# SewoongLab/PLeaS-Merging

Measured on NVIDIA B200. Metric: rn50_pair_merge_calib_samples_per_s, higher is better.
Workload: dtype f32

## Files before the change

include/pleas_b200.h:

```cpp
#ifndef PLEAS_B200_H
#define PLEAS_B200_H

#include <stdint.h>

#ifdef __cplusplus
extern "C" {
#endif

#define PLB_OK 0
#define PLB_EINVAL (-1)
#define PLB_ESIZE (-2)
#define PLB_EALIGN (-3)

#define PLB_MODE_INNER 0
#define PLB_MODE_NEG_CDIST 1
#define PLB_MODE_CORR 2

int plb_version(void);
const char *plb_last_error_string(void);


int64_t plb_plane_bytes(int64_t rows, int64_t K, int32_t *row_groups, int32_t *k_blocks);

int plb_pack_split(const float *x, int64_t outer, int64_t src_rows, int64_t inner,
// ... 53 lines not shown
  const double *qa, *qb;
  const double *sa, *sb;
  int64_t ld_m, ld_n, K;
  int32_t splits;
  int32_t n_affine;
  const double *affine;
} PlbFinalizeTap;
typedef struct PlbFinalizeGroup {
  float *cost;
  int64_t ldc;
  int32_t n, tap_begin, tap_end, block_begin;
} PlbFinalizeGroup;
int plb_cross_finalize_grouped(const PlbFinalizeTap *taps_dev, const PlbFinalizeGroup *groups_dev,
                               int32_t n_groups, int32_t total_blocks, int32_t mode, int32_t accumulate,
                               void *stream);

int plb_cross_finalize_corr(const float *partial, int32_t splits, int64_t ld_m, int64_t ld_n,
                            int64_t M, int64_t N, const double *qa, const double *qb,
                            const double *sa, const double *sb, int64_t K, float *cost, int64_t ldc,
                            int32_t accumulate, void *stream);

int plb_lap_solve_batched(const float *const *cost, const int32_t *n, const int32_t *ld,
                          int64_t *const *col4row, double *objective, int32_t *status,
                          int32_t n_problems, int32_t max_n, int32_t maximize, void *stream);

int plb_lap_solve_batched_warm(const float *const *cost, const int32_t *n, const int32_t *ld,
                               int64_t *const *col4row, double *objective, int32_t *status,
                               int32_t n_problems, int32_t max_n, int32_t maximize,
                               const double *const *v_in, double v_scale, double *const *v_out, void *stream);


int plb_get_blocks(const float *cost, int64_t ldc, const int64_t *perm, int32_t n, float ratio,
                   int32_t identity, int64_t *q_merged, int64_t *p_merged, int64_t *q_sep,
                   int64_t *p_sep, int32_t *counts, void *stream);

int plb_block_merge(const float *w1, const float *w2, int64_t O, int64_t I, int64_t R,
                    const int64_t *bo1, const int64_t *bo2, const int64_t *bo1c, const int64_t *bo2c,
                    int64_t no, int64_t mo,
                    const int64_t *bi1, const int64_t *bi2, const int64_t *bi1c, const int64_t *bi2c,
                    int64_t ni, int64_t mi, int32_t in_axis_only, float *out, void *stream);

int plb_gather_axis(const float *in, float *out, int64_t outer, int64_t n, int64_t inner,
                    const int64_t *P, void *stream);

int plb_compose_perm(const int64_t *a, const int64_t *b, int64_t *out, int64_t n, void *stream);

int plb_wm_progress(const float *A, int64_t ld, const int64_t *P, int32_t n, int32_t *flag,
                    double *gain, void *stream);

int plb_conv_debug_set_trace(unsigned long long *dev_buf);
int64_t plb_conv_packed_floats(int64_t Cout, int64_t Cin, int32_t KH, int32_t KW);
int plb_conv_pack_weights(const float *w, int64_t Cout, int64_t Cin, int32_t KH, int32_t KW, float *packed,
                          void *stream);

int plb_conv2d_forward(const float *const *x, const float *const *packed_w, const float *const *bias,
                       float *const *out, int32_t nprob, int64_t NB, int64_t Cin, int64_t IH, int64_t IW,
                       int64_t Cout, int32_t KH, int32_t KW, int32_t stride, int32_t pad_h, int32_t pad_w,
                       void *stream);

int plb_conv2d_affine_forward(const float *const *x, const float *const *packed_w, const float *const *bias,
                              float *const *out, const float *const *scale_shift, float *const *out2,
                              int32_t relu, int32_t nprob, int64_t NB, int64_t Cin, int64_t IH, int64_t IW,
                              int64_t Cout, int32_t KH, int32_t KW, int32_t stride, int32_t pad_h, int32_t pad_w,
                              void *stream);

int plb_chol_solve(double *G, int64_t n, double *B, int64_t nrhs, double ridge, int32_t *info,
                   void *stream);

#ifdef __cplusplus
}
#endif
#endif
```

pleas_merging_b200/_native.py:

```python
import ctypes
import os

_HERE = os.path.dirname(os.path.abspath(__file__))
LIB_PATH = os.path.join(_HERE, "lib", "libpleas_b200.so")

c_i32, c_i64, c_f32, c_f64, c_ptr = ctypes.c_int32, ctypes.c_int64, ctypes.c_float, ctypes.c_double, ctypes.c_void_p


class GemmProblem(ctypes.Structure):
    _fields_ = [
        ("a_hi", c_ptr), ("a_lo", c_ptr), ("b_hi", c_ptr), ("b_lo", c_ptr), ("partial", c_ptr),
        ("a_row_groups", c_i32), ("b_row_groups", c_i32), ("k_blocks", c_i32),
        ("m_tiles", c_i32), ("n_tiles", c_i32), ("splits", c_i32), ("cta_begin", c_i32), ("symmetric", c_i32),
    ]


class FinalizeTap(ctypes.Structure):
    _fields_ = [("partial", c_ptr), ("qa", c_ptr), ("qb", c_ptr), ("sa", c_ptr), ("sb", c_ptr),
                ("ld_m", c_i64), ("ld_n", c_i64), ("K", c_i64), ("splits", c_i32), ("n_affine", c_i32),
                ("affine", c_ptr)]


class FinalizeGroup(ctypes.Structure):
    _fields_ = [("cost", c_ptr), ("ldc", c_i64), ("n", c_i32), ("tap_begin", c_i32), ("tap_end", c_i32),
                ("block_begin", c_i32)]


_SIGNATURES = {
    "plb_version": (ctypes.c_int, []),
    "plb_last_error_string": (ctypes.c_char_p, []),
    "plb_plane_bytes": (c_i64, [c_i64, c_i64, ctypes.POINTER(c_i32), ctypes.POINTER(c_i32)]),
    "plb_pack_split": (ctypes.c_int, [c_ptr, c_i64, c_i64, c_i64, c_ptr, c_i64, c_ptr, c_ptr, c_i32, c_i32,
                                      c_ptr, c_ptr, c_ptr]),
    "plb_pack_split_pair": (ctypes.c_int, [c_ptr, c_ptr, c_i64, c_i64, c_i64, c_ptr, c_ptr, c_ptr, c_ptr, c_i32, c_i32,
                                           c_ptr, c_ptr, c_ptr]),
    "plb_gram_direct": (ctypes.c_int, [c_ptr, c_ptr, c_i64, c_i64, c_i64, c_ptr, c_i32, c_i32, c_ptr, c_ptr, c_ptr]),
    "plb_gram_tma": (ctypes.c_int, [c_ptr, c_ptr, c_i64, c_i64, c_i64, c_ptr, c_i32, c_i32, c_ptr, c_ptr, c_ptr, c_ptr,
                                    c_ptr]),
    "plb_pack_split_pair_sums": (ctypes.c_int, [c_ptr, c_ptr, c_i64, c_i64, c_i64, c_ptr, c_ptr, c_ptr, c_ptr, c_i32,
                                                c_i32, c_ptr, c_ptr, c_ptr, c_ptr, c_ptr]),
    "plb_cross_finalize_grouped": (ctypes.c_int, [c_ptr, c_ptr, c_i32, c_i32, c_i32, c_i32, c_ptr]),
    "plb_cross_finalize_corr": (ctypes.c_int, [c_ptr, c_i32, c_i64, c_i64, c_i64, c_i64, c_ptr, c_ptr, c_ptr, c_ptr,
                                               c_i64, c_ptr, c_i64, c_i32, c_ptr]),
    "plb_gram_tma_geometry": (ctypes.c_int, [c_i64, ctypes.POINTER(c_i32), ctypes.POINTER(c_i32),
                                             ctypes.POINTER(c_i32), ctypes.POINTER(c_i32), ctypes.POINTER(c_i32)]),
    "plb_debug_set_trace": (ctypes.c_int, [c_ptr]),
    "plb_pack_im2col": (ctypes.c_int, [c_ptr, c_ptr, c_i64, c_i64, c_i64, c_i64, c_ptr, c_ptr, c_ptr, c_ptr, c_i64,
                                       c_i32, c_i32, c_i32, c_i32, c_i32, c_i32, c_i32, c_i32, c_i64, c_i64, c_i32,
                                       c_ptr, c_ptr, c_i32, c_i32, c_ptr]),
    "plb_gemm_grouped": (ctypes.c_int, [c_ptr, c_i32, c_i32, c_i32, c_i32, c_ptr]),
    "plb_cross_finalize": (ctypes.c_int, [c_ptr, c_i32, c_i64, c_i64, c_i64, c_i64, c_ptr, c_ptr, c_i32, c_ptr,
                                          c_ptr, c_i64, c_i32, c_i32, c_ptr]),
    "plb_lap_solve_batched": (ctypes.c_int, [c_ptr, c_ptr, c_ptr, c_ptr, c_ptr, c_ptr, c_i32, c_i32, c_i32, c_ptr]),
    "plb_lap_solve_batched_warm": (ctypes.c_int, [c_ptr, c_ptr, c_ptr, c_ptr, c_ptr, c_ptr, c_i32, c_i32, c_i32, c_ptr,
                                                  c_f64, c_ptr, c_ptr]),
    "plb_get_blocks": (ctypes.c_int, [c_ptr, c_i64, c_ptr, c_i32, c_f32, c_i32, c_ptr, c_ptr, c_ptr, c_ptr, c_ptr,
                                      c_ptr]),
    "plb_block_merge": (ctypes.c_int, [c_ptr, c_ptr, c_i64, c_i64, c_i64, c_ptr, c_ptr, c_ptr, c_ptr, c_i64, c_i64,
                                       c_ptr, c_ptr, c_ptr, c_ptr, c_i64, c_i64, c_i32, c_ptr, c_ptr]),
    "plb_gather_axis": (ctypes.c_int, [c_ptr, c_ptr, c_i64, c_i64, c_i64, c_ptr, c_ptr]),
    "plb_compose_perm": (ctypes.c_int, [c_ptr, c_ptr, c_ptr, c_i64, c_ptr]),
    "plb_wm_progress": (ctypes.c_int, [c_ptr, c_i64, c_ptr, c_i32, c_ptr, c_ptr, c_ptr]),
    "plb_chol_solve": (ctypes.c_int, [c_ptr, c_i64, c_ptr, c_i64, c_f64, c_ptr, c_ptr]),
    "plb_conv_debug_set_trace": (ctypes.c_int, [c_ptr]),
    "plb_conv_packed_floats": (c_i64, [c_i64, c_i64, c_i32, c_i32]),
    "plb_conv_pack_weights": (ctypes.c_int, [c_ptr, c_i64, c_i64, c_i32, c_i32, c_ptr, c_ptr]),
    "plb_conv2d_forward": (ctypes.c_int, [c_ptr, c_ptr, c_ptr, c_ptr, c_i32, c_i64, c_i64, c_i64, c_i64, c_i64,
                                          c_i32, c_i32, c_i32, c_i32, c_i32, c_ptr]),
    "plb_conv2d_affine_forward": (ctypes.c_int, [c_ptr, c_ptr, c_ptr, c_ptr, c_ptr, c_ptr, c_i32, c_i32, c_i64, c_i64,
                                                 c_i64, c_i64, c_i64, c_i32, c_i32, c_i32, c_i32, c_i32, c_ptr]),
}

EXPORTED_SYMBOLS = tuple(_SIGNATURES)
_lib = None


def lib():
    global _lib
    if _lib is None:
        if not os.path.exists(LIB_PATH):
            raise RuntimeError(
                f"pleas_merging_b200: CUDA library not found at {LIB_PATH}; build it with "
                "`python -m pleas_merging_b200.build` (or __graft_entry__.build()). There is no CPU fallback.")
        handle = ctypes.CDLL(LIB_PATH)
        for name, (res, args) in _SIGNATURES.items():
            fn = getattr(handle, name)
            fn.restype, fn.argtypes = res, args
        _lib = handle
    return _lib


import collections

LAUNCH_COUNTS = collections.Counter()


def check(rc, what):
    LAUNCH_COUNTS[what] += 1
    if rc != 0:
        msg = lib().plb_last_error_string().decode(errors="replace")
        raise RuntimeError(f"pleas_merging_b200: {what} failed with status {rc}: {msg}")


def call(name, device, *args):
    import torch

    fn = getattr(lib(), name)
    if device.index is None or device.index == torch.cuda.current_device():
        rc = fn(*args, torch.cuda.current_stream().cuda_stream)
    else:
        with torch.cuda.device(device):
            rc = fn(*args, torch.cuda.current_stream(device).cuda_stream)
    check(rc, name)


def stream_ptr(device=None):
    import torch

    return torch.cuda.current_stream(device).cuda_stream
# ... 17 lines not shown
```

pleas_merging_b200/csrc/conv.cu:

```cuda
#include "tma.cuh"

namespace plb {

constexpr int kConvStages = 4;
constexpr int kConvThreads = 576;
constexpr int kConvMaxFlatK = 512;

struct ConvParams {
  const float *x[2];
  const float *bias[2];
  float *out[2];
  const float2 *post[2];
  float *out2[2];
  int post_relu;
  int nprob;
  int NB, Cin, IH, IW, Cout, OH, OW, KH, KW, stride, pad_h, pad_w;
  int P, OHW, IHW;
  int m_tiles, n_tiles, total_items;
  int taps;
  int nbox;
  int flat;
  int flat_groups;
  int flat_lg;
  int chain_boxes;
  unsigned long long *trace;
  int debug;
};

__device__ __forceinline__ void tmem_st16(uint32_t taddr, const uint32_t (&v)[16]) {
  asm volatile(
      "tcgen05.st.sync.aligned.32x32b.x16.b32 [%0], "
      "{%1, %2, %3, %4, %5, %6, %7, %8, %9, %10, %11, %12, %13, %14, %15, %16};" ::"r"(taddr),
      "r"(v[0]), "r"(v[1]), "r"(v[2]), "r"(v[3]), "r"(v[4]), "r"(v[5]), "r"(v[6]), "r"(v[7]), "r"(v[8]), "r"(v[9]),
      "r"(v[10]), "r"(v[11]), "r"(v[12]), "r"(v[13]), "r"(v[14]), "r"(v[15])
      : "memory");
}
__device__ __forceinline__ void tmem_st_wait() { asm volatile("tcgen05.wait::st.sync.aligned;" ::: "memory"); }
__device__ __forceinline__ void tmem_ld16(uint32_t taddr, uint32_t (&v)[16]) {
  asm volatile(
      "tcgen05.ld.sync.aligned.32x32b.x16.b32 "
      "{%0, %1, %2, %3, %4, %5, %6, %7, %8, %9, %10, %11, %12, %13, %14, %15}, [%16];"
      : "=r"(v[0]), "=r"(v[1]), "=r"(v[2]), "=r"(v[3]), "=r"(v[4]), "=r"(v[5]), "=r"(v[6]), "=r"(v[7]),
        "=r"(v[8]), "=r"(v[9]), "=r"(v[10]), "=r"(v[11]), "=r"(v[12]), "=r"(v[13]), "=r"(v[14]), "=r"(v[15])
      : "r"(taddr));
}
__device__ __forceinline__ void umma_tf32_ts(uint32_t tmem_d, uint32_t tmem_a, uint64_t bdesc, uint32_t idesc,
                                             uint32_t accumulate) {
  asm volatile(
      "{\n\t.reg .pred p;\n\t"
      "setp.ne.b32 p, %4, 0;\n\t"
      "tcgen05.mma.cta_group::1.kind::tf32 [%0], [%1], %2, %3, p;\n\t}" ::"r"(tmem_d),
      "r"(tmem_a), "l"(bdesc), "r"(idesc), "r"(accumulate)
      : "memory");
}
__device__ __forceinline__ void tma_load_4d(void *smem_dst, const CUtensorMap *map, int c0, int c1, int c2, int c3,
                                            uint64_t *bar) {
  asm volatile(
      "cp.async.bulk.tensor.4d.shared::cluster.global.tile.mbarrier::complete_tx::bytes [%0], [%1, {%2, %3, %4, %5}], "
      "[%6];" ::"r"(smem_u32(smem_dst)),
      "l"(map), "r"(c0), "r"(c1), "r"(c2), "r"(c3), "r"(smem_u32(bar))
      : "memory");
}

template <int TN>
struct ConvCfg {
  static constexpr int kBBytes = kConvStages * 2 * TN * 128;
  static constexpr int kARing = TN == 128 ? 5 : 8;
  static constexpr int kSmemBytes = kBBytes + kARing * 16384 + 1024;
};

__device__ __forceinline__ void cp_async4(uint32_t smem_dst, const float *src, uint32_t ignore) {
  asm volatile(
      "{\n\t.reg .pred p;\n\t"
      "setp.ne.b32 p, %2, 0;\n\t"
      "cp.async.ca.shared.global [%0], [%1], 4, p;\n\t}" ::"r"(smem_dst),
      "l"(src), "r"(ignore)
      : "memory");
}
__device__ __forceinline__ void cp_async_commit() { asm volatile("cp.async.commit_group;" ::: "memory"); }
template <int N>
__device__ __forceinline__ void cp_async_wait() {
  asm volatile("cp.async.wait_group %0;" ::"n"(N) : "memory");
}

__device__ __forceinline__ uint32_t opaque_smem_u32(const void *p) {
  uint32_t a;
  asm volatile("{\n\t.reg .u64 t;\n\tcvta.to.shared.u64 t, %1;\n\tcvt.u32.u64 %0, t;\n\t}" : "=r"(a) : "l"(p));
  return a;
}
__device__ __forceinline__ void a32_expect_tx(uint32_t bar, uint32_t bytes) {
  asm volatile("mbarrier.arrive.expect_tx.shared::cta.b64 _, [%0], %1;" ::"r"(bar), "r"(bytes) : "memory");
}
__device__ __forceinline__ void a32_arrive(uint32_t bar) {
  asm volatile("mbarrier.arrive.shared::cta.b64 _, [%0];" ::"r"(bar) : "memory");
}
__device__ __forceinline__ bool a32_try_wait(uint32_t bar, uint32_t parity) {
  uint32_t ok;
  asm volatile(
      "{\n\t.reg .pred P;\n\t"
      "mbarrier.try_wait.parity.shared::cta.b64 P, [%1], %2;\n\t"
      "selp.b32 %0, 1, 0, P;\n\t}"
      : "=r"(ok)
      : "r"(bar), "r"(parity)
      : "memory");
  return ok != 0;
}
__device__ __forceinline__ bool a32_test_wait(uint32_t bar, uint32_t parity) {
  uint32_t ok;
  asm volatile(
      "{\n\t.reg .pred P;\n\t"
      "mbarrier.test_wait.parity.shared::cta.b64 P, [%1], %2;\n\t"
      "selp.b32 %0, 1, 0, P;\n\t}"
      : "=r"(ok)
      : "r"(bar), "r"(parity)
      : "memory");
  return ok != 0;
}
__device__ __forceinline__ void a32_wait_wd(uint32_t bar, uint32_t parity) {
  if (a32_try_wait(bar, parity)) return;
  const long long t0 = clock64();
  while (!a32_try_wait(bar, parity))
    if (clock64() - t0 > kWatchdogClocks) __trap();
// ... 19 lines not shown
    const int2 e = rows[r];
    const bool rowok = pvalid && e.y >= 0 && (unsigned)(ih0 + e.y) < (unsigned)IH;
    const float *base = rowok ? origin + e.x : safe;
#pragma unroll
    for (int t = 0; t < TAPS; ++t) {
      const bool ok = rowok && t < KW && (unsigned)(iw0 + t) < (unsigned)IW;
      cp_async4(dst + (r * TAPS + t) * 512, base + (ok ? t : 0), ok ? 0u : 1u);
    }
  }
}

template <int COLS, bool BIAS, bool POST>
__device__ __forceinline__ void store_tile(const float (&acc)[COLS], float *o, float *o2, int ohw, const float *bias,
                                           const float2 *ss, bool relu, int) {
#pragma unroll
  for (int c = 0; c < COLS; ++c) {
    const float v = acc[c];
    o[(int64_t)c * ohw] = v;
    if (POST) {
      const float2 a = __ldg(ss + c);
      const float w = fmaf(v, a.x, a.y);
      o2[(int64_t)c * ohw] = relu ? fmaxf(w, 0.f) : w;
    }
  }
}
template <int COLS>
__device__ __noinline__ void store_tile_ragged(const float (&acc)[COLS], float *o, float *o2, int ohw, const float *bias,
                                               const float2 *ss, bool relu, int nc) {
#pragma unroll 4
  for (int c = 0; c < COLS; ++c) {
    if (c >= nc) break;
    const float v = acc[c] + (bias ? __ldg(bias + c) : 0.f);
    o[(int64_t)c * ohw] = v;
    if (o2 != nullptr) {
      const float2 a = __ldg(ss + c);
      const float w = fmaf(v, a.x, a.y);
      o2[(int64_t)c * ohw] = relu ? fmaxf(w, 0.f) : w;
    }
  }
}

struct ConvItem {
  int prob, mt, nt;
};
__device__ __forceinline__ ConvItem conv_item(const ConvParams &p, int item) {
  ConvItem it;
  it.nt = item % p.n_tiles;
  const int rest = item / p.n_tiles;
  it.prob = rest % p.nprob;
  it.mt = rest / p.nprob;
  return it;
}

template <int TN, int CH, bool DBG>
__global__ void __launch_bounds__(kConvThreads, 1) conv3xtf32_kernel(const __grid_constant__ CUtensorMap tmw0,
                                                                      const __grid_constant__ CUtensorMap tmw1,
                                                                      ConvParams p) {
  constexpr int kPlaneBytes = TN * 128;
  constexpr int kStageBytes = 2 * kPlaneBytes;
  constexpr uint32_t kACol0 = 2 * TN;
  constexpr int kARing = ConvCfg<TN>::kARing;
  extern __shared__ uint8_t smem_raw[];
  __shared__ uint64_t bars[2 * kConvStages + 4];
  __shared__ uint32_t tmem_base_s;
  __shared__ int2 ktab[kConvMaxFlatK];

  uint8_t *smem = (uint8_t *)(((uintptr_t)smem_raw + 1023) & ~(uintptr_t)1023);
  const int warp = threadIdx.x >> 5, lane = threadIdx.x & 31;
  const int cta = (int)blockIdx.x, nctas = (int)gridDim.x;
  const uint32_t bars_a = opaque_smem_u32(bars), smem_a = opaque_smem_u32(smem);
  const uint32_t bar_full = bars_a, bar_empty = bars_a + 8 * kConvStages, bar_acc_full = bars_a + 16 * kConvStages,
                 bar_acc_empty = bar_acc_full + 16;

  if (warp == 0 && lane == 0) {
    for (int s = 0; s < kConvStages; ++s) {
      mbar_init(&bars[s], 1 + 8);
      mbar_init(&bars[kConvStages + s], 1);
    }
    for (int b = 0; b < 2; ++b) {
      mbar_init(&bars[2 * kConvStages + b], 1);
      mbar_init(&bars[2 * kConvStages + 2 + b], 8);
    }
    fence_mbar_init();
  } else if (warp == 1) {
    tmem_alloc(&tmem_base_s, 512);
    tmem_relinquish();
  }
  if (p.flat) {
    const int rows = (p.nbox * 32) >> p.flat_lg;
    for (int g = (int)threadIdx.x; g < rows; g += kConvThreads) {
      int2 e;
      if (g < p.flat_groups) {
        const int ci = g / p.KH, kh = g - ci * p.KH;
        e.x = ci * p.IHW + kh * p.IW;
        e.y = kh;
      } else {
        e.x = 0;
        e.y = -1;
      }
      ktab[g] = e;
    }
  }
  tc_fence_before();
  __syncthreads();
  tc_fence_after();
  const uint32_t tmem_base = tmem_base_s;

  if (warp == 0) {
    uint32_t i = 0;
    for (int item = cta; item < p.total_items; item += nctas) {
      const ConvItem it = conv_item(p, item);
      const CUtensorMap *map = it.prob ? &tmw1 : &tmw0;
      const int n0 = it.nt * TN;
      int cb = 0, tap = 0;
      for (int b = 0; b < p.nbox; ++b, ++i) {
        const uint32_t s = i & (kConvStages - 1), ph = (i / kConvStages) & 1u;
        a32_wait_wd(bar_empty + 8 * s, ph ^ 1u);
        if (DBG && p.trace && cta == 0 && lane == 0 && i < 512) p.trace[i * 16 + 0] = clock64();
        if (elect_one()) {
          const uint32_t st = smem_a + s * kStageBytes;
          a32_expect_tx(bar_full + 8 * s, kStageBytes);
          a32_tma_load_4d(st, map, cb * 32, n0, tap, 0, bar_full + 8 * s);
          a32_tma_load_4d(st + kPlaneBytes, map, cb * 32, n0, tap, 1, bar_full + 8 * s);
        }
        __syncwarp();
        if (++tap == p.taps) {
          tap = 0;
          ++cb;
        }
      }
    }
  } else if (warp == 1) {
    constexpr uint32_t idesc = umma_idesc_tf32(128, TN);
    const uint32_t smem_base = smem_a;
    uint32_t i = 0, chain = 0;
    uint32_t ready = 0;
    bool acc_ok = false;
    for (int item = cta; item < p.total_items; item += nctas) {
      for (int b0 = 0; b0 < p.nbox; b0 += CH, ++chain) {
        const uint32_t buf = chain & 1u;
        const int nb = min(CH, p.nbox - b0);
// ... 9 lines not shown
        if (elect_one()) {
#pragma unroll
          for (int q = 0; q < CH; ++q) {
            if (q >= nb) break;
            const uint32_t s = (i + q) & (kConvStages - 1);
            const uint32_t bst = smem_base + s * kStageBytes, a_hi0 = tmem_base + kACol0 + s * 64;
#pragma unroll
            for (int j = 0; j < 4; ++j) {
              umma_tf32_ts(d_tmem, a_hi0 + 32 + 8 * j, umma_desc_sw<128>(bst + 32 * j), idesc, (q > 0 || j > 0) ? 1u : 0u);
              if (!(DBG && p.debug & 2))
                umma_tf32_ts(d_tmem, a_hi0 + 8 * j, umma_desc_sw<128>(bst + kPlaneBytes + 32 * j), idesc, 1u);
            }
          }
        }
        __syncwarp();
        uint32_t nready = 0;
#pragma unroll
        for (int q = 0; q < CH; ++q) {
          const uint32_t in = i + nb + q;
          if (a32_test_wait(bar_full + 8 * (in & (kConvStages - 1)), (in / kConvStages) & 1u)) nready |= 1u << q;
        }
        const bool next_acc = a32_test_wait(bar_acc_empty + 8 * ((chain + 1) & 1u), (((chain + 1) >> 1) & 1u) ^ 1u);
        if (elect_one()) {
#pragma unroll
          for (int q = 0; q < CH; ++q) {
            if (q >= nb) break;
            const uint32_t s = (i + q) & (kConvStages - 1);
            const uint32_t bst = smem_base + s * kStageBytes, a_hi0 = tmem_base + kACol0 + s * 64;
            if (!(DBG && p.debug & 2)) {
#pragma unroll
              for (int j = 0; j < 4; ++j) umma_tf32_ts(d_tmem, a_hi0 + 8 * j, umma_desc_sw<128>(bst + 32 * j), idesc, 1u);
            }
            a32_commit(bar_empty + 8 * s);
          }
          a32_commit(bar_acc_full + 8 * buf);
        }
        ready = __reduce_and_sync(0xffffffffu, nready);
        acc_ok = __all_sync(0xffffffffu, next_acc);
        if (trm) p.trace[i * 16 + 6] = clock64();
        i += nb;
      }
    }
  } else if (warp < 10) {
    const int hsel = (warp - 2) >> 2;
    const int row = (warp & 3) * 32 + lane;
    const uint32_t a_base = tmem_base + ((uint32_t)((warp & 3) * 32) << 16) + kACol0 + 16 * hsel;
    const uint32_t ring = smem_a + ConvCfg<TN>::kBBytes + (uint32_t)(hsel * 16) * 512u + (uint32_t)row * 4u;
    const int my_items = cta < p.total_items ? (p.total_items - cta + nctas - 1) / nctas : 0;
    const int total = my_items * p.nbox;
    const int kh_n = p.flat ? 1 : p.KH, kw_n = p.flat ? 1 : p.KW, cb_n = p.nbox / (kh_n * kw_n);
    int itx = 0, cb = 0, kh = 0, kw = 0, ih0 = 0, iw0 = 0;
    bool pvalid = false;
    const float *xn = nullptr;
    auto locate = [&]() {
      const ConvItem it = conv_item(p, cta + itx * nctas);
      const int pos = it.mt * 128 + row;
      pvalid = pos < p.P;
      const int n = pvalid ? pos / p.OHW : 0, r = pos - n * p.OHW, oh = r / p.OW, ow = r - oh * p.OW;
      ih0 = oh * p.stride - p.pad_h;
      iw0 = ow * p.stride - p.pad_w;
      xn = p.x[it.prob] + (int64_t)n * p.Cin * p.IHW;
    };
    if (total > 0) locate();

    auto issue = [&](int slot) {
      const uint32_t dst = ring + (uint32_t)slot * 16384u;
      if (!p.flat) {
        const int ih = ih0 + kh, iw = iw0 + kw;
        const bool ok = pvalid && (unsigned)ih < (unsigned)p.IH && (unsigned)iw < (unsigned)p.IW;
        const float *src = ok ? xn + (int64_t)(cb * 32 + hsel * 16) * p.IHW + ih * p.IW + iw : xn;
        const uint32_t cs = ok ? (uint32_t)p.IHW : 0u, ign = ok ? 0u : 1u;
#pragma unroll
        for (int c = 0; c < 16; ++c) cp_async4(dst + c * 512, src + (uint32_t)c * cs, ign);
      } else {
        const int row0 = (cb * 32 + hsel * 16) >> p.flat_lg;
        const float *origin = xn + ih0 * p.IW + iw0;
        switch (p.flat_lg) {
          case 0: flat_rows<0>(ktab + row0, origin, xn, dst, pvalid, ih0, iw0, p.IH, p.IW, p.KW); break;
          case 1: flat_rows<1>(ktab + row0, origin, xn, dst, pvalid, ih0, iw0, p.IH, p.IW, p.KW); break;
          case 2: flat_rows<2>(ktab + row0, origin, xn, dst, pvalid, ih0, iw0, p.IH, p.IW, p.KW); break;
          case 3: flat_rows<3>(ktab + row0, origin, xn, dst, pvalid, ih0, iw0, p.IH, p.IW, p.KW); break;
          default: flat_rows<4>(ktab + row0, origin, xn, dst, pvalid, ih0, iw0, p.IH, p.IW, p.KW); break;
        }
      }
      if (++kw == kw_n) {
        kw = 0;
        if (++kh == kh_n) {
          kh = 0;
          if (++cb == cb_n) {
            cb = 0;
            ++itx;
            if (itx < my_items) locate();
          }
        }
      }
    };

    int slot_in = 0;
#pragma unroll 1
    for (int j = 0; j < kARing - 1; ++j) {
      if (j < total && !(DBG && p.debug & 1)) issue(slot_in);
      cp_async_commit();
      if (++slot_in == kARing) slot_in = 0;
    }
    int slot_out = 0;
#pragma unroll 1
    for (int i = 0; i < total; ++i) {
      if (i + kARing - 1 < total && !(DBG && p.debug & 1)) issue(slot_in);
      cp_async_commit();
      if (++slot_in == kARing) slot_in = 0;
      cp_async_wait<kARing - 1>();
      uint32_t v[16];
#pragma unroll
      for (int c = 0; c < 16; ++c)
        asm volatile("ld.shared.b32 %0, [%1];" : "=r"(v[c]) : "r"(ring + (uint32_t)slot_out * 16384u + c * 512u) : "memory");
      if (++slot_out == kARing) slot_out = 0;
      const uint32_t s = (uint32_t)i & (kConvStages - 1), ph = ((uint32_t)i / kConvStages) & 1u;
      const bool tr = DBG && p.trace && cta == 0 && warp == 2 && lane == 0 && i < 512;
      a32_wait_wd(bar_empty + 8 * s, ph ^ 1u);
      tc_fence_after();
      uint32_t hi[16];
#pragma unroll
      for (int c = 0; c < 16; ++c) hi[c] = (v[c] + 0x1000u) & 0xffffe000u;
      tmem_st16(a_base + s * 64, hi);
#pragma unroll
      for (int c = 0; c < 16; ++c)
        hi[c] = __float_as_uint(__uint_as_float(v[c]) - __uint_as_float(hi[c])) + 0x1000u;
      tmem_st16(a_base + s * 64 + 32, hi);
      tmem_st_wait();
      if (tr) p.trace[i * 16 + 3] = clock64();
      tc_fence_before();
      __syncwarp();
      if (lane == 0) a32_arrive(bar_full + 8 * s);
    }
  } else {
    constexpr int COLS = TN / 2;
    const int q = warp & 3;
    const int half = (warp - 10) >> 2;
    uint32_t chain = 0;
    for (int item = cta; item < p.total_items; item += nctas) {
      const ConvItem it = conv_item(p, item);
      unsigned long long acc2[COLS / 2];
#pragma unroll
      for (int c = 0; c < COLS / 2; ++c) acc2[c] = 0ull;
      for (int b0 = 0; b0 < p.nbox; b0 += CH, ++chain) {
        const uint32_t buf = chain & 1u;
        a32_wait_wd(bar_acc_full + 8 * buf, (chain >> 1) & 1u);
        const bool tr = DBG && p.trace && cta == 0 && warp == 10 && lane == 0 && chain < 512;
        if (tr) p.trace[chain * 16 + 5] = clock64();
        tc_fence_after();
        const uint32_t t0 = tmem_base + ((uint32_t)(q * 32) << 16) + buf * TN + half * COLS;
#pragma unroll
        for (int c = 0; c < COLS / 16; ++c) {
          uint32_t v[16];
          tmem_ld16(t0 + c * 16, v);
          tmem_ld_wait();
#pragma unroll
          for (int e = 0; e < 8; ++e) {
            unsigned long long pr;
            asm("mov.b64 %0, {%1, %2};" : "=l"(pr) : "r"(v[2 * e]), "r"(v[2 * e + 1]));
            asm("add.rn.f32x2 %0, %0, %1;" : "+l"(acc2[c * 8 + e]) : "l"(pr));
          }
        }
        tc_fence_before();
        __syncwarp();
        if (lane == 0) a32_arrive(bar_acc_empty + 8 * buf);
        if (tr) p.trace[chain * 16 + 7] = clock64();
      }
      float acc[COLS];
#pragma unroll
      for (int c = 0; c < COLS / 2; ++c) {
        uint32_t lo, hi;
        asm("mov.b64 {%0, %1}, %2;" : "=r"(lo), "=r"(hi) : "l"(acc2[c]));
        acc[2 * c] = __uint_as_float(lo);
        acc[2 * c + 1] = __uint_as_float(hi);
      }
      const int pos = it.mt * 128 + q * 32 + lane;
      if (pos < p.P && !(DBG && p.debug & 4)) {
        const int n = pos / p.OHW, r = pos - n * p.OHW;
        const int co0 = it.nt * TN + half * COLS;
        float *o = p.out[it.prob] + ((int64_t)n * p.Cout + co0) * p.OHW + r;
        const float *bias = p.bias[it.prob];
        const int ohw = p.OHW;
        const int nc = min(COLS, p.Cout - co0);
        float *o2 = p.out2[it.prob] ? p.out2[it.prob] + ((int64_t)n * p.Cout + co0) * p.OHW + r : nullptr;
        const float2 *ss = p.post[it.prob] ? p.post[it.prob] + co0 : nullptr;
        const bool relu = p.post_relu != 0;
        if (nc == COLS && bias == nullptr && o2 == nullptr) {
          store_tile<COLS, false, false>(acc, o, o2, ohw, bias, ss, relu, nc);
        } else if (nc == COLS && bias == nullptr) {
          store_tile<COLS, false, true>(acc, o, o2, ohw, bias, ss, relu, nc);
        } else {
          store_tile_ragged<COLS>(acc, o, o2, ohw, bias ? bias + co0 : nullptr, ss, relu, nc);
        }
      }
    }
  }

  tc_fence_before();
  __syncthreads();
  if (warp == 1) tmem_dealloc(tmem_base, 512);
}

__global__ void conv_pack_weights_kernel(const float *__restrict__ w, float *__restrict__ packed, int Cout, int Cin,
                                         int KH, int KW, int taps, int Kc, int flat, int flat_lg) {
  const int64_t plane = (int64_t)taps * Cout * Kc;
  for (int64_t idx = (int64_t)blockIdx.x * blockDim.x + threadIdx.x; idx < plane; idx += (int64_t)gridDim.x * blockDim.x) {
    const int k = (int)(idx % Kc);
    const int co = (int)((idx / Kc) % Cout);
    const int t = (int)(idx / ((int64_t)Kc * Cout));
    float v = 0.f;
    if (!flat) {
      v = w[((int64_t)co * Cin + k) * (KH * KW) + t];
    } else {
      const int g = k >> flat_lg, kw = k & ((1 << flat_lg) - 1);
      if (g < Cin * KH && kw < KW) v = w[((int64_t)co * Cin * KH + g) * KW + kw];
    }
    const float hi = to_tf32(v);
    packed[idx] = hi;
    packed[plane + idx] = to_tf32(v - hi);
  }
}

static unsigned long long *g_conv_trace = nullptr;

struct ConvGeometry {
  int flat, taps, Kc, flat_lg;
};
static ConvGeometry conv_geometry(int64_t Cin, int KH, int KW) {
  ConvGeometry g;
  g.flat = (Cin % 32) != 0;
  g.taps = g.flat ? 1 : KH * KW;
  g.flat_lg = 0;
  while ((1 << g.flat_lg) < KW) ++g.flat_lg;
  g.Kc = g.flat ? (int)(ceil_div((Cin * KH) << g.flat_lg, 32) * 32) : (int)Cin;
  return g;
}

static int make_weight_map(CUtensorMap *m, const float *packed, int64_t Cout, const ConvGeometry &g, int tn) {
  EncodeTiledFn enc = encode_tiled();
  PLB_REQUIRE(enc != nullptr, PLB_EINVAL, "plb_conv2d_forward: cuTensorMapEncodeTiled is not available from this driver");
  cuuint64_t gdim[4] = {(cuuint64_t)g.Kc, (cuuint64_t)Cout, (cuuint64_t)g.taps, 2};
  cuuint64_t gstride[3] = {(cuuint64_t)g.Kc * 4, (cuuint64_t)g.Kc * Cout * 4, (cuuint64_t)g.Kc * Cout * g.taps * 4};
  cuuint32_t box[4] = {32, (cuuint32_t)tn, 1, 1};
  cuuint32_t estr[4] = {1, 1, 1, 1};
  CUresult r = enc(m, CU_TENSOR_MAP_DATA_TYPE_FLOAT32, 4, (void *)packed, gdim, gstride, box, estr,
                   CU_TENSOR_MAP_INTERLEAVE_NONE, CU_TENSOR_MAP_SWIZZLE_128B, CU_TENSOR_MAP_L2_PROMOTION_L2_256B,
                   CU_TENSOR_MAP_FLOAT_OOB_FILL_NONE);
  PLB_REQUIRE(r == CUDA_SUCCESS, PLB_EINVAL, "plb_conv2d_forward: cuTensorMapEncodeTiled failed with CUresult %d", (int)r);
  return PLB_OK;
}

template <int TN, int CH, bool DBG>
static int launch_conv(const CUtensorMap &m0, const CUtensorMap &m1, const ConvParams &p, cudaStream_t stream) {
  constexpr int smem_bytes = ConvCfg<TN>::kSmemBytes;
  if (int rc = ensure_dynamic_smem((const void *)conv3xtf32_kernel<TN, CH, DBG>, smem_bytes, "conv3xtf32_kernel"))
    return rc;
  const int grid = min(p.total_items, device_sm_count());
  conv3xtf32_kernel<TN, CH, DBG><<<grid, kConvThreads, smem_bytes, stream>>>(m0, m1, p);
  return launch_status("conv3xtf32_kernel");
}

}

extern "C" int plb_conv_debug_set_trace(unsigned long long *dev_buf) {
  plb::g_conv_trace = dev_buf;
  return PLB_OK;
}

extern "C" int64_t plb_conv_packed_floats(int64_t Cout, int64_t Cin, int32_t KH, int32_t KW) {
  if (Cout <= 0 || Cin <= 0 || KH <= 0 || KW <= 0) return 0;
  const plb::ConvGeometry g = plb::conv_geometry(Cin, KH, KW);
  return 2ll * g.taps * Cout * g.Kc;
}

extern "C" int plb_conv_pack_weights(const float *w, int64_t Cout, int64_t Cin, int32_t KH, int32_t KW, float *packed,
                                     void *stream) {
  using namespace plb;
  PLB_REQUIRE(w && packed, PLB_EINVAL, "plb_conv_pack_weights: null pointer");
  PLB_REQUIRE(Cout > 0 && Cin > 0 && KH > 0 && KW > 0, PLB_EINVAL, "plb_conv_pack_weights: empty weight");
  const ConvGeometry g = conv_geometry(Cin, KH, KW);
  PLB_REQUIRE(!g.flat || KW <= 16, PLB_ESIZE, "plb_conv_pack_weights: Cin %% 32 != 0 needs KW <= 16");
  PLB_REQUIRE(!g.flat || g.Kc <= kConvMaxFlatK, PLB_ESIZE,
              "plb_conv_pack_weights: Cin %% 32 != 0 needs Cin*KH*pow2(KW) <= %d", kConvMaxFlatK);
  const int64_t plane = (int64_t)g.taps * Cout * g.Kc;
  PLB_REQUIRE(plane < (1ll << 31), PLB_ESIZE, "plb_conv_pack_weights: weight too large");
  const int64_t want = ceil_div(plane, 256);
  const int blocks = (int)(want < 148 * 8 ? want : 148 * 8);
  conv_pack_weights_kernel<<<blocks, 256, 0, (cudaStream_t)stream>>>(w, packed, (int)Cout, (int)Cin, KH, KW, g.taps,
                                                                     g.Kc, g.flat, g.flat_lg);
  return launch_status("conv_pack_weights_kernel");
}

extern "C" int plb_conv2d_forward(const float *const *x, const float *const *packed_w, const float *const *bias,
                                  float *const *out, int32_t nprob, int64_t NB, int64_t Cin, int64_t IH, int64_t IW,
                                  int64_t Cout, int32_t KH, int32_t KW, int32_t stride, int32_t pad_h, int32_t pad_w,
                                  void *stream) {
  return plb_conv2d_affine_forward(x, packed_w, bias, out, nullptr, nullptr, 0, nprob, NB, Cin, IH, IW, Cout, KH, KW,
                                   stride, pad_h, pad_w, stream);
}

extern "C" int plb_conv2d_affine_forward(const float *const *x, const float *const *packed_w,
                                         const float *const *bias, float *const *out,
                                         const float *const *scale_shift, float *const *out2, int32_t relu,
                                         int32_t nprob, int64_t NB, int64_t Cin, int64_t IH, int64_t IW, int64_t Cout,
                                         int32_t KH, int32_t KW, int32_t stride, int32_t pad_h, int32_t pad_w,
                                         void *stream) {
  using namespace plb;
  PLB_REQUIRE(x && packed_w && out, PLB_EINVAL, "plb_conv2d_forward: null pointer table");
  PLB_REQUIRE(nprob == 1 || nprob == 2, PLB_EINVAL, "plb_conv2d_forward: one or two problems per launch");
  PLB_REQUIRE(NB > 0 && Cin > 0 && IH > 0 && IW > 0 && Cout > 0 && KH > 0 && KW > 0 && stride > 0 && pad_h >= 0 &&
                  pad_w >= 0,
              PLB_EINVAL, "plb_conv2d_forward: bad geometry");
  const int64_t OH = (IH + 2 * pad_h - KH) / stride + 1, OW = (IW + 2 * pad_w - KW) / stride + 1;
  PLB_REQUIRE(OH > 0 && OW > 0, PLB_EINVAL, "plb_conv2d_forward: empty output");
  PLB_REQUIRE(NB * OH * OW < (1ll << 31) - 128 && NB * Cin * IH * IW < (1ll << 40) && Cin * IH * IW < (1ll << 31) &&
                  KH < 256 && KW < 256,
              PLB_ESIZE, "plb_conv2d_forward: extent too large");
  const ConvGeometry g = conv_geometry(Cin, KH, KW);
  PLB_REQUIRE(!g.flat || KW <= 16, PLB_ESIZE, "plb_conv2d_forward: Cin %% 32 != 0 needs KW <= 16");
  PLB_REQUIRE(!g.flat || g.Kc <= kConvMaxFlatK, PLB_ESIZE,
              "plb_conv2d_forward: Cin %% 32 != 0 needs Cin*KH*pow2(KW) <= %d", kConvMaxFlatK);
  ConvParams p = {};
  for (int i = 0; i < nprob; ++i) {
    PLB_REQUIRE(x[i] && packed_w[i] && out[i], PLB_EINVAL, "plb_conv2d_forward: null pointer");
    PLB_REQUIRE(((uintptr_t)packed_w[i] & 15) == 0, PLB_EALIGN, "plb_conv2d_forward: packed weights must be 16-byte aligned");
    p.x[i] = x[i];
    p.out[i] = out[i];
    p.bias[i] = bias ? bias[i] : nullptr;
    PLB_REQUIRE((scale_shift == nullptr) == (out2 == nullptr) &&
                    (out2 == nullptr || ((scale_shift[i] != nullptr) && (out2[i] != nullptr))),
                PLB_EINVAL, "plb_conv2d_affine_forward: scale_shift and out2 go together");
    PLB_REQUIRE(scale_shift == nullptr || ((uintptr_t)scale_shift[i] & 7) == 0, PLB_EALIGN,
                "plb_conv2d_affine_forward: scale_shift must be 8-byte aligned");
    p.post[i] = scale_shift ? reinterpret_cast<const float2 *>(scale_shift[i]) : nullptr;
    p.out2[i] = out2 ? out2[i] : nullptr;
  }
  p.nprob = nprob;
  p.post_relu = relu;
  p.NB = (int)NB, p.Cin = (int)Cin, p.IH = (int)IH, p.IW = (int)IW, p.Cout = (int)Cout, p.OH = (int)OH, p.OW = (int)OW;
  p.KH = KH, p.KW = KW, p.stride = stride, p.pad_h = pad_h, p.pad_w = pad_w;
  p.P = (int)(NB * OH * OW), p.OHW = (int)(OH * OW), p.IHW = (int)(IH * IW);
  p.flat = g.flat, p.taps = g.taps, p.flat_groups = (int)(Cin * KH), p.flat_lg = g.flat_lg;
  p.nbox = g.taps * (g.Kc / 32);
  static int debug = -1;
  if (debug < 0) {
    const char *d = getenv("PLB_CONV_DEBUG");
    debug = d ? atoi(d) : 0;
  }
  p.debug = debug;
  p.trace = g_conv_trace;
  static int chain = 0;
  if (chain == 0) {
    const char *c = getenv("PLB_CONV_CHAIN");
    chain = (c && atoi(c) > 0 && atoi(c) <= kConvStages / 2) ? atoi(c) : 2;
  }
  p.chain_boxes = chain;
  const int tn = Cout <= 64 ? 64 : 128;
  p.m_tiles = (int)ceil_div(p.P, 128);
  p.n_tiles = (int)ceil_div(Cout, tn);
  const int64_t items = (int64_t)p.m_tiles * p.n_tiles * nprob;
  PLB_REQUIRE(items * p.nbox < (1ll << 31), PLB_ESIZE, "plb_conv2d_forward: too many work items");
  p.total_items = (int)items;
  CUtensorMap m0, m1;
  if (int rc = make_weight_map(&m0, packed_w[0], Cout, g, tn)) return rc;
  if (int rc = make_weight_map(&m1, packed_w[nprob - 1], Cout, g, tn)) return rc;
  cudaStream_t s = (cudaStream_t)stream;
  const bool dbg = p.debug != 0 || p.trace != nullptr;
  if (dbg || chain != 2) {
    if (chain == 1) return tn == 64 ? launch_conv<64, 1, true>(m0, m1, p, s) : launch_conv<128, 1, true>(m0, m1, p, s);
    return tn == 64 ? launch_conv<64, 2, true>(m0, m1, p, s) : launch_conv<128, 2, true>(m0, m1, p, s);
  }
  return tn == 64 ? launch_conv<64, 2, false>(m0, m1, p, s) : launch_conv<128, 2, false>(m0, m1, p, s);
}
```

Measured before the change: 2705.

## Add windowed-input conv kernel with TMA/bulk-loaded halo windows in shared memory

Adds a window variant of the tcgen05 conv kernel for stride-1 'same' convolutions with Cin divisible by 32. An extra producer warp bulk-copies (or, for 1x1 convs, TMA-loads) a contiguous 128-pixel window plus halo per 32-channel block into a shared-memory ring. The A-operand warps then read every kh/kw tap from that window with predicated shared loads instead of issuing per-tap cp.async gathers from global memory. This cuts redundant global/L2 traffic and per-element async-copy overhead, at the cost of a new smem ring, more barriers, an extra warp, and extra complexity in the edge handling.

Result: faster. 2779 (median of 6 runs) (+2.7%).

```diff
diff --git a/include/pleas_b200.h b/include/pleas_b200.h
--- a/include/pleas_b200.h
+++ b/include/pleas_b200.h
@@ -129,6 +129,8 @@
 int64_t plb_conv_packed_floats(int64_t Cout, int64_t Cin, int32_t KH, int32_t KW);
 int plb_conv_pack_weights(const float *w, int64_t Cout, int64_t Cin, int32_t KH, int32_t KW, float *packed,
                           void *stream);
+int32_t plb_conv_route(const float *const *x, int32_t nprob, int64_t Cin, int64_t IH, int64_t IW, int32_t KH,
+                       int32_t KW, int32_t stride, int32_t pad_h, int32_t pad_w);
 
 int plb_conv2d_forward(const float *const *x, const float *const *packed_w, const float *const *bias,
                        float *const *out, int32_t nprob, int64_t NB, int64_t Cin, int64_t IH, int64_t IW,
diff --git a/pleas_merging_b200/_native.py b/pleas_merging_b200/_native.py
--- a/pleas_merging_b200/_native.py
+++ b/pleas_merging_b200/_native.py
@@ -65,6 +65,7 @@
     "plb_conv_debug_set_trace": (ctypes.c_int, [c_ptr]),
     "plb_conv_packed_floats": (c_i64, [c_i64, c_i64, c_i32, c_i32]),
     "plb_conv_pack_weights": (ctypes.c_int, [c_ptr, c_i64, c_i64, c_i32, c_i32, c_ptr, c_ptr]),
+    "plb_conv_route": (c_i32, [c_ptr, c_i32, c_i64, c_i64, c_i64, c_i32, c_i32, c_i32, c_i32, c_i32]),
     "plb_conv2d_forward": (ctypes.c_int, [c_ptr, c_ptr, c_ptr, c_ptr, c_i32, c_i64, c_i64, c_i64, c_i64, c_i64,
                                           c_i32, c_i32, c_i32, c_i32, c_i32, c_ptr]),
     "plb_conv2d_affine_forward": (ctypes.c_int, [c_ptr, c_ptr, c_ptr, c_ptr, c_ptr, c_ptr, c_i32, c_i32, c_i64, c_i64,
diff --git a/pleas_merging_b200/csrc/conv.cu b/pleas_merging_b200/csrc/conv.cu
--- a/pleas_merging_b200/csrc/conv.cu
+++ b/pleas_merging_b200/csrc/conv.cu
@@ -4,6 +4,10 @@
 
 constexpr int kConvStages = 4;
 constexpr int kConvThreads = 576;
+constexpr int kConvWinThreads = kConvThreads + 32;
+constexpr int kConvWinMaxLen = 256;
+constexpr int kConvWinMaxStages = 8;
+constexpr int kConvSmemOptin = 227 * 1024;
 constexpr int kConvMaxFlatK = 512;
 
 struct ConvParams {
@@ -23,6 +27,11 @@
   int flat_groups;
   int flat_lg;
   int chain_boxes;
+  int win_h;
+  int win_len;
+  int win_stages;
+  int win_tma;
+  int win_sub;
   unsigned long long *trace;
   int debug;
 };
@@ -68,6 +77,21 @@
   static constexpr int kARing = TN == 128 ? 5 : 8;
   static constexpr int kSmemBytes = kBBytes + kARing * 16384 + 1024;
 };
+
+__device__ __forceinline__ void a32_tma_load_3d(uint32_t smem_dst, const CUtensorMap *map, int c0, int c1, int c2,
+                                                uint32_t bar) {
+  asm volatile(
+      "cp.async.bulk.tensor.3d.shared::cluster.global.tile.mbarrier::complete_tx::bytes [%0], [%1, {%2, %3, %4}], [%5];" ::
+          "r"(smem_dst),
+      "l"(map), "r"(c0), "r"(c1), "r"(c2), "r"(bar)
+      : "memory");
+}
+__device__ __forceinline__ void bulk_g2s(uint32_t smem_dst, const float *src, uint32_t bytes, uint32_t bar) {
+  asm volatile(
+      "cp.async.bulk.shared::cluster.global.mbarrier::complete_tx::bytes [%0], [%1], %2, [%3];" ::"r"(smem_dst),
+      "l"(src), "r"(bytes), "r"(bar)
+      : "memory");
+}
 
 __device__ __forceinline__ void cp_async4(uint32_t smem_dst, const float *src, uint32_t ignore) {
   asm volatile(
@@ -193,16 +217,15 @@
   return it;
 }
 
-template <int TN, int CH, bool DBG>
-__global__ void __launch_bounds__(kConvThreads, 1) conv3xtf32_kernel(const __grid_constant__ CUtensorMap tmw0,
-                                                                      const __grid_constant__ CUtensorMap tmw1,
-                                                                      ConvParams p) {
+template <int TN, int CH, bool DBG, bool WIN>
+__device__ __forceinline__ void conv3xtf32_body(const CUtensorMap &tmw0, const CUtensorMap &tmw1, const CUtensorMap &tmx0,
+                                                const CUtensorMap &tmx1, const ConvParams &p) {
   constexpr int kPlaneBytes = TN * 128;
   constexpr int kStageBytes = 2 * kPlaneBytes;
   constexpr uint32_t kACol0 = 2 * TN;
   constexpr int kARing = ConvCfg<TN>::kARing;
   extern __shared__ uint8_t smem_raw[];
-  __shared__ uint64_t bars[2 * kConvStages + 4];
+  __shared__ uint64_t bars[2 * kConvStages + 4 + (WIN ? 2 * kConvWinMaxStages : 0)];
   __shared__ uint32_t tmem_base_s;
   __shared__ int2 ktab[kConvMaxFlatK];
 
@@ -211,7 +234,8 @@
   const int cta = (int)blockIdx.x, nctas = (int)gridDim.x;
   const uint32_t bars_a = opaque_smem_u32(bars), smem_a = opaque_smem_u32(smem);
   const uint32_t bar_full = bars_a, bar_empty = bars_a + 8 * kConvStages, bar_acc_full = bars_a + 16 * kConvStages,
-                 bar_acc_empty = bar_acc_full + 16;
+                 bar_acc_empty = bar_acc_full + 16, bar_win_full = bar_acc_full + 32,
+                 bar_win_free = bar_win_full + 8 * kConvWinMaxStages;
 
   if (warp == 0 && lane == 0) {
     for (int s = 0; s < kConvStages; ++s) {
@@ -222,12 +246,18 @@
       mbar_init(&bars[2 * kConvStages + b], 1);
       mbar_init(&bars[2 * kConvStages + 2 + b], 8);
     }
+    if (WIN) {
+      for (int s = 0; s < kConvWinMaxStages; ++s) {
+        mbar_init(&bars[2 * kConvStages + 4 + s], 1);
+        mbar_init(&bars[2 * kConvStages + 4 + kConvWinMaxStages + s], 8);
+      }
+    }
     fence_mbar_init();
   } else if (warp == 1) {
     tmem_alloc(&tmem_base_s, 512);
     tmem_relinquish();
   }
-  if (p.flat) {
+  if (!WIN && p.flat) {
     const int rows = (p.nbox * 32) >> p.flat_lg;
     for (int g = (int)threadIdx.x; g < rows; g += kConvThreads) {
       int2 e;
@@ -343,6 +373,8 @@
     int itx = 0, cb = 0, kh = 0, kw = 0, ih0 = 0, iw0 = 0;
     bool pvalid = false;
     const float *xn = nullptr;
+    const uint32_t wcs = (uint32_t)p.win_len * 4u;
+    uint32_t wsub = 0;
     auto locate = [&]() {
       const ConvItem it = conv_item(p, cta + itx * nctas);
       const int pos = it.mt * 128 + row;
@@ -351,9 +383,22 @@
       ih0 = oh * p.stride - p.pad_h;
       iw0 = ow * p.stride - p.pad_w;
       xn = p.x[it.prob] + (int64_t)n * p.Cin * p.IHW;
+      if (WIN && p.win_tma && pvalid) wsub = (uint32_t)(n - it.mt * 128 / p.IHW) * 32u * wcs;
     };
     if (total > 0) locate();
 
+    auto advance = [&]() {
+      if (++kw < kw_n) return false;
+      kw = 0;
+      if (++kh < kh_n) return false;
+      kh = 0;
+      if (++cb == cb_n) {
+        cb = 0;
+        ++itx;
+        if (itx < my_items) locate();
+      }
+      return true;
+    };
     auto issue = [&](int slot) {
       const uint32_t dst = ring + (uint32_t)slot * 16384u;
       if (!p.flat) {
@@ -374,38 +419,50 @@
           default: flat_rows<4>(ktab + row0, origin, xn, dst, pvalid, ih0, iw0, p.IH, p.IW, p.KW); break;
         }
       }
-      if (++kw == kw_n) {
-        kw = 0;
-        if (++kh == kh_n) {
-          kh = 0;
-          if (++cb == cb_n) {
-            cb = 0;
-            ++itx;
-            if (itx < my_items) locate();
-          }
-        }
-      }
+      advance();
     };
 
-    int slot_in = 0;
+    int slot_in = 0, slot_out = 0;
+    if (!WIN) {
 #pragma unroll 1
-    for (int j = 0; j < kARing - 1; ++j) {
-      if (j < total && !(DBG && p.debug & 1)) issue(slot_in);
-      cp_async_commit();
-      if (++slot_in == kARing) slot_in = 0;
-    }
-    int slot_out = 0;
+      for (int j = 0; j < kARing - 1; ++j) {
+        if (j < total && !(DBG && p.debug & 1)) issue(slot_in);
+        cp_async_commit();
+        if (++slot_in == kARing) slot_in = 0;
+      }
+    }
+    const uint32_t wst = (uint32_t)p.win_sub * 32u * wcs;
+    const uint32_t win0 = smem_a + ConvCfg<TN>::kBBytes + (uint32_t)(hsel * 16) * wcs + (uint32_t)(p.win_h + row) * 4u;
+    uint32_t wslot = 0, wph = 0;
 #pragma unroll 1
     for (int i = 0; i < total; ++i) {
-      if (i + kARing - 1 < total && !(DBG && p.debug & 1)) issue(slot_in);
-      cp_async_commit();
-      if (++slot_in == kARing) slot_in = 0;
-      cp_async_wait<kARing - 1>();
       uint32_t v[16];
-#pragma unroll
-      for (int c = 0; c < 16; ++c)
-        asm volatile("ld.shared.b32 %0, [%1];" : "=r"(v[c]) : "r"(ring + (uint32_t)slot_out * 16384u + c * 512u) : "memory");
-      if (++slot_out == kARing) slot_out = 0;
+      bool block_done = false;
+      if (WIN) {
+        if (kh == 0 && kw == 0) a32_wait_wd(bar_win_full + 8 * wslot, wph);
+        const int ih = ih0 + kh, iw = iw0 + kw;
+        const uint32_t ok = pvalid && (unsigned)ih < (unsigned)p.IH && (unsigned)iw < (unsigned)p.IW;
+        const uint32_t src = win0 + wslot * wst + wsub + (uint32_t)(((kh - p.pad_h) * p.IW + kw - p.pad_w) * 4);
+#pragma unroll
+        for (int c = 0; c < 16; ++c) {
+          v[c] = 0u;
+          asm volatile(
+              "{\n\t.reg .pred q;\n\tsetp.ne.b32 q, %2, 0;\n\t@q ld.shared.b32 %0, [%1];\n\t}"
+              : "+r"(v[c])
+              : "r"(src + c * wcs), "r"(ok)
+              : "memory");
+        }
+        block_done = advance();
+      } else {
+        if (i + kARing - 1 < total && !(DBG && p.debug & 1)) issue(slot_in);
+        cp_async_commit();
+        if (++slot_in == kARing) slot_in = 0;
+        cp_async_wait<kARing - 1>();
+#pragma unroll
+        for (int c = 0; c < 16; ++c)
+          asm volatile("ld.shared.b32 %0, [%1];" : "=r"(v[c]) : "r"(ring + (uint32_t)slot_out * 16384u + c * 512u) : "memory");
+        if (++slot_out == kARing) slot_out = 0;
+      }
       const uint32_t s = (uint32_t)i & (kConvStages - 1), ph = ((uint32_t)i / kConvStages) & 1u;
       const bool tr = DBG && p.trace && cta == 0 && warp == 2 && lane == 0 && i < 512;
       a32_wait_wd(bar_empty + 8 * s, ph ^ 1u);
@@ -423,8 +480,15 @@
       tc_fence_before();
       __syncwarp();
       if (lane == 0) a32_arrive(bar_full + 8 * s);
-    }
-  } else {
+      if (WIN && block_done) {
+        if (lane == 0) a32_arrive(bar_win_free + 8 * wslot);
+        if (++wslot == (uint32_t)p.win_stages) {
+          wslot = 0;
+          wph ^= 1u;
+        }
+      }
+    }
+  } else if (!WIN || warp < kConvThreads / 32) {
     constexpr int COLS = TN / 2;
     const int q = warp & 3;
     const int half = (warp - 10) >> 2;
@@ -486,11 +550,64 @@
         }
       }
     }
+  } else {
+    const int hw = p.IHW, cb_n = p.Cin / 32;
+    const uint32_t wcs = (uint32_t)p.win_len * 4u, wst = (uint32_t)p.win_sub * 32u * wcs;
+    const uint32_t dst0 = smem_a + ConvCfg<TN>::kBBytes + (uint32_t)lane * wcs;
+    uint32_t wslot = 0, wph = 0;
+    for (int item = cta; item < p.total_items; item += nctas) {
+      const ConvItem it = conv_item(p, item);
+      const int wlo = it.mt * 128 - p.win_h;
+      const int w0 = max(wlo, 0), w1 = min(it.mt * 128 + 128 + p.win_h, p.P);
+      const float *xc = p.x[it.prob] + (int64_t)lane * hw;
+      const CUtensorMap *xmap = it.prob ? &tmx1 : &tmx0;
+      const int n0 = w0 / hw, nimg = (w1 - 1) / hw - n0 + 1;
+      for (int cb = 0; cb < cb_n; ++cb, xc += (int64_t)32 * hw) {
+        a32_wait_wd(bar_win_free + 8 * wslot, wph ^ 1u);
+        if (p.win_tma) {
+          if (elect_one()) {
+            a32_expect_tx(bar_win_full + 8 * wslot, (uint32_t)nimg * 16384u);
+            for (int j = 0; j < nimg; ++j)
+              a32_tma_load_3d(smem_a + ConvCfg<TN>::kBBytes + wslot * wst + (uint32_t)j * 32u * wcs, xmap,
+                              w0 - (n0 + j) * hw, cb * 32, n0 + j, bar_win_full + 8 * wslot);
+          }
+          __syncwarp();
+        } else {
+          if (lane == 0) a32_expect_tx(bar_win_full + 8 * wslot, (uint32_t)(w1 - w0) * 128u);
+          __syncwarp();
+          for (int a = w0, n = w0 / hw; a < w1; ++n) {
+            const int e = min(w1, (n + 1) * hw);
+            bulk_g2s(dst0 + wslot * wst + (uint32_t)(a - wlo) * 4u, xc + (int64_t)n * p.Cin * hw + (a - n * hw),
+                     (uint32_t)(e - a) * 4u, bar_win_full + 8 * wslot);
+            a = e;
+          }
+        }
+        if (++wslot == (uint32_t)p.win_stages) {
+          wslot = 0;
+          wph ^= 1u;
+        }
+      }
+    }
   }
 
   tc_fence_before();
   __syncthreads();
   if (warp == 1) tmem_dealloc(tmem_base, 512);
+}
+
+template <int TN, int CH, bool DBG>
+__global__ void __launch_bounds__(kConvThreads, 1) conv3xtf32_kernel(const __grid_constant__ CUtensorMap tmw0,
+                                                                      const __grid_constant__ CUtensorMap tmw1,
+                                                                      ConvParams p) {
+  conv3xtf32_body<TN, CH, DBG, false>(tmw0, tmw1, tmw0, tmw1, p);
+}
+template <int TN, int CH, bool DBG>
+__global__ void __launch_bounds__(kConvWinThreads, 1) conv3xtf32_window_kernel(const __grid_constant__ CUtensorMap tmw0,
+                                                                               const __grid_constant__ CUtensorMap tmw1,
+                                                                               const __grid_constant__ CUtensorMap tmx0,
+                                                                               const __grid_constant__ CUtensorMap tmx1,
+                                                                               ConvParams p) {
+  conv3xtf32_body<TN, CH, DBG, true>(tmw0, tmw1, tmx0, tmx1, p);
 }
 
 __global__ void conv_pack_weights_kernel(const float *__restrict__ w, float *__restrict__ packed, int Cout, int Cin,
@@ -542,6 +659,17 @@
   return PLB_OK;
 }
 
+static int conv_window_len(const float *const *x, int nprob, int64_t Cin, int64_t IH, int64_t IW, int KH, int KW,
+                           int stride, int pad_h, int pad_w) {
+  if (Cin % 32 != 0 || stride != 1 || KH != 2 * pad_h + 1 || KW != 2 * pad_w + 1 || (IH * IW) % 4 != 0 ||
+      (KH * KW == 1 && IH * IW < 128))
+    return 0;
+  for (int i = 0; i < nprob; ++i)
+    if (((uintptr_t)x[i] & 15) != 0) return 0;
+  const int64_t halo = (pad_h * IW + pad_w + 3) / 4 * 4;
+  return 128 + 2 * halo <= kConvWinMaxLen ? (int)(128 + 2 * halo) : 0;
+}
+
 template <int TN, int CH, bool DBG>
 static int launch_conv(const CUtensorMap &m0, const CUtensorMap &m1, const ConvParams &p, cudaStream_t stream) {
   constexpr int smem_bytes = ConvCfg<TN>::kSmemBytes;
@@ -550,6 +678,52 @@
   const int grid = min(p.total_items, device_sm_count());
   conv3xtf32_kernel<TN, CH, DBG><<<grid, kConvThreads, smem_bytes, stream>>>(m0, m1, p);
   return launch_status("conv3xtf32_kernel");
+}
+
+static int make_input_map(CUtensorMap *m, const float *x, const ConvParams &p) {
+  EncodeTiledFn enc = encode_tiled();
+  PLB_REQUIRE(enc != nullptr, PLB_EINVAL, "plb_conv2d_forward: cuTensorMapEncodeTiled is not available from this driver");
+  cuuint64_t gdim[3] = {(cuuint64_t)p.IHW, (cuuint64_t)p.Cin, (cuuint64_t)p.NB};
+  cuuint64_t gstride[2] = {(cuuint64_t)p.IHW * 4, (cuuint64_t)p.IHW * p.Cin * 4};
+  cuuint32_t box[3] = {128, 32, 1};
+  cuuint32_t estr[3] = {1, 1, 1};
+  CUresult r = enc(m, CU_TENSOR_MAP_DATA_TYPE_FLOAT32, 3, (void *)x, gdim, gstride, box, estr, CU_TENSOR_MAP_INTERLEAVE_NONE,
+                   CU_TENSOR_MAP_SWIZZLE_NONE, CU_TENSOR_MAP_L2_PROMOTION_L2_256B, CU_TENSOR_MAP_FLOAT_OOB_FILL_NONE);
+  PLB_REQUIRE(r == CUDA_SUCCESS, PLB_EINVAL, "plb_conv2d_forward: cuTensorMapEncodeTiled (x) failed with CUresult %d", (int)r);
+  return PLB_OK;
+}
+
+template <int TN, int CH, bool DBG>
+static int launch_conv_window(const CUtensorMap &m0, const CUtensorMap &m1, ConvParams p, cudaStream_t stream) {
+  const void *fn = (const void *)conv3xtf32_window_kernel<TN, CH, DBG>;
+  static int static_bytes = -1;
+  if (static_bytes < 0) {
+    cudaFuncAttributes a;
+    const cudaError_t e = cudaFuncGetAttributes(&a, fn);
+    PLB_REQUIRE(e == cudaSuccess, (int)e, "cudaFuncGetAttributes(conv3xtf32_window_kernel): %s", cudaGetErrorString(e));
+    static_bytes = (int)a.sharedSizeBytes;
+  }
+  CUtensorMap x0 = m0, x1 = m1;
+  p.win_tma = p.KH * p.KW == 1;
+  p.win_sub = p.win_tma ? 2 : 1;
+  if (p.win_tma) {
+    if (int rc = make_input_map(&x0, p.x[0], p)) return rc;
+    if (int rc = make_input_map(&x1, p.x[p.nprob - 1], p)) return rc;
+  }
+  const int stage_bytes = p.win_sub * 128 * p.win_len;
+  const int room = kConvSmemOptin - static_bytes - 1024 - ConvCfg<TN>::kBBytes;
+  p.win_stages = min(kConvWinMaxStages, room / stage_bytes);
+  PLB_REQUIRE(p.win_stages >= 2, PLB_ESIZE, "plb_conv2d_forward: window ring of %d stages", p.win_stages);
+  const int smem_bytes = ConvCfg<TN>::kBBytes + p.win_stages * stage_bytes + 1024;
+  if (int rc = ensure_dynamic_smem(fn, smem_bytes, "conv3xtf32_window_kernel")) return rc;
+  const int grid = min(p.total_items, device_sm_count());
+  conv3xtf32_window_kernel<TN, CH, DBG><<<grid, kConvWinThreads, smem_bytes, stream>>>(m0, m1, x0, x1, p);
+  return launch_status("conv3xtf32_window_kernel");
+}
+
+template <int TN, int CH, bool DBG>
+static int launch_route(const CUtensorMap &m0, const CUtensorMap &m1, const ConvParams &p, cudaStream_t stream) {
+  return p.win_len ? launch_conv_window<TN, CH, DBG>(m0, m1, p, stream) : launch_conv<TN, CH, DBG>(m0, m1, p, stream);
 }
 
 }
@@ -634,6 +808,8 @@
   p.P = (int)(NB * OH * OW), p.OHW = (int)(OH * OW), p.IHW = (int)(IH * IW);
   p.flat = g.flat, p.taps = g.taps, p.flat_groups = (int)(Cin * KH), p.flat_lg = g.flat_lg;
   p.nbox = g.taps * (g.Kc / 32);
+  p.win_len = conv_window_len(x, nprob, Cin, IH, IW, KH, KW, stride, pad_h, pad_w);
+  p.win_h = p.win_len ? (p.win_len - 128) / 2 : 0;
   static int debug = -1;
   if (debug < 0) {
     const char *d = getenv("PLB_CONV_DEBUG");
@@ -659,8 +835,16 @@
   cudaStream_t s = (cudaStream_t)stream;
   const bool dbg = p.debug != 0 || p.trace != nullptr;
   if (dbg || chain != 2) {
-    if (chain == 1) return tn == 64 ? launch_conv<64, 1, true>(m0, m1, p, s) : launch_conv<128, 1, true>(m0, m1, p, s);
-    return tn == 64 ? launch_conv<64, 2, true>(m0, m1, p, s) : launch_conv<128, 2, true>(m0, m1, p, s);
-  }
-  return tn == 64 ? launch_conv<64, 2, false>(m0, m1, p, s) : launch_conv<128, 2, false>(m0, m1, p, s);
-}
+    if (chain == 1) return tn == 64 ? launch_route<64, 1, true>(m0, m1, p, s) : launch_route<128, 1, true>(m0, m1, p, s);
+    return tn == 64 ? launch_route<64, 2, true>(m0, m1, p, s) : launch_route<128, 2, true>(m0, m1, p, s);
+  }
+  return tn == 64 ? launch_route<64, 2, false>(m0, m1, p, s) : launch_route<128, 2, false>(m0, m1, p, s);
+}
+
+extern "C" int32_t plb_conv_route(const float *const *x, int32_t nprob, int64_t Cin, int64_t IH, int64_t IW,
+                                  int32_t KH, int32_t KW, int32_t stride, int32_t pad_h, int32_t pad_w) {
+  if (x == nullptr || nprob < 1 || nprob > 2 || Cin <= 0 || IH <= 0 || IW <= 0 || KH <= 0 || KW <= 0 || stride <= 0 ||
+      pad_h < 0 || pad_w < 0)
+    return PLB_EINVAL;
+  return plb::conv_window_len(x, nprob, Cin, IH, IW, KH, KW, stride, pad_h, pad_w) > 0 ? 1 : 0;
+}
```
